# Justin900429/autonomous_driving_with_diffusion_model

Measured on AMD Instinct MI355X. Metric: denoising-steps/sec, higher is better.
Workload: dtype f32

## Files before the change

autonomous_driving_with_diffusion_model_amd/_lib.py:

```python
from __future__ import annotations

import ctypes as C
import os
from typing import Optional, Sequence

import torch

_HERE = os.path.dirname(os.path.abspath(__file__))
LIB_PATH = os.environ.get("ADX_LIB") or os.path.join(_HERE, "libadx.so")

c_f32p = C.POINTER(C.c_float)
i32, i64, f32, vp = C.c_int32, C.c_int64, C.c_float, C.c_void_p


class TConvDesc(C.Structure):
    _fields_ = [("kind", i32), ("taps", i32), ("stride", i32), ("pad", i32), ("c0", i32), ("c1", i32),
                ("cout", i32), ("lin", i32), ("lout", i32), ("groups", i32), ("eps", f32), ("w_layout", i32),
                ("w_flip", i32), ("exact", i32), ("lin_valid", i32), ("lout_valid", i32)]


class TConvIO(C.Structure):
    _fields_ = [("x0", vp), ("x0_sb", i64), ("x0_sc", i64), ("x0_sl", i64),
                ("x1", vp), ("x1_sb", i64), ("x1_sc", i64), ("x1_sl", i64),
                ("packed_w", vp), ("bias", vp), ("gamma", vp), ("beta", vp),
# ... 64 lines not shown
    "adx_resnet_forward": (i32, [vp, vp, vp, vp, i32, i32, i32, vp, vp]),
    "adx_resnet_forward_u8": (i32, [vp, vp, vp, vp, C.POINTER(C.c_float), C.POINTER(C.c_float), i32, i32, i32, vp, vp]),
    "adx_resnet_tape_create": (i32, [C.POINTER(vp)]),
    "adx_resnet_tape_destroy": (None, [vp]),
    "adx_resnet_train_workspace_bytes": (C.c_size_t, [vp, i32, i32, i32]),
    "adx_resnet_forward_train": (i32, [vp, C.POINTER(vp), i32, vp, vp, C.c_size_t, vp, i32, i32, i32, vp, vp, i32, vp]),
    "adx_resnet_backward": (i32, [vp, C.POINTER(vp), C.POINTER(vp), i32, vp, C.c_size_t, vp, vp, vp]),
    "adx_resnet_backward_groups": (i32, [vp]),
    "adx_resnet_tensor_group": (i32, [vp, i32]),
    "adx_resnet_backward_events": (i32, [vp, C.POINTER(vp), C.POINTER(vp), i32, vp, C.c_size_t, vp, vp, C.POINTER(vp), i32, vp]),
    "adx_conv2d_packed_bytes": (C.c_size_t, [C.POINTER(Conv2dDesc)]),
    "adx_conv2d_pack": (i32, [C.POINTER(Conv2dDesc), vp, vp, vp]),
    "adx_conv2d_forward": (i32, [C.POINTER(Conv2dDesc), vp, vp, vp, vp, vp, vp, i32, i32, i32, i32, vp]),
    "adx_conv2d_cells_supported": (i32, [C.POINTER(Conv2dDesc), i32, i32, i32]),
    "adx_conv2d_forward_cells": (i32, [C.POINTER(Conv2dDesc), vp, vp, vp, vp, vp, vp, i32, i32, i32, i32, i32, vp]),
    "adx_conv2d_wgrad_scratch_bytes": (C.c_size_t, []),
    "adx_conv2d_wgrad": (i32, [C.POINTER(Conv2dDesc), vp, vp, vp, i32, i32, i32, vp, vp]),
    "adx_conv2d_wgrad_ex": (i32, [C.POINTER(Conv2dDesc), vp, vp, vp, i32, i32, i32, vp, i32, vp]),
    "adx_conv2d_wgrad_cells": (i32, [C.POINTER(Conv2dDesc), vp, vp, vp, vp, i32, i32, i32, vp, vp]),
    "adx_trajpred_create": (i32, [i32, C.POINTER(vp)]),
    "adx_trajpred_destroy": (None, [vp]),
    "adx_trajpred_num_params": (i32, [vp]),
    "adx_trajpred_packed_bytes": (C.c_size_t, [vp]),
    "adx_trajpred_scratch_bytes": (C.c_size_t, [vp, i32, i32]),
    "adx_trajpred_set_scratch": (i32, [vp, vp, C.c_size_t]),
    "adx_trajpred_pack": (i32, [vp, C.POINTER(vp), i32, vp, vp, vp]),
    "adx_trajpred_forward": (i32, [vp, vp, vp, i64, i64, vp, vp, i32, i32, vp]),
    "adx_trajpred_backward": (i32, [vp, vp, vp, i64, i64, vp, vp, vp, i32, i32, vp]),
    "adx_trajpred_backward_params": (i32, [vp, vp, vp, i64, i64, vp, vp, vp, vp, vp, i32, i32, C.c_float, C.c_uint64, vp]),
    "adx_trajpred_forward_train": (i32, [vp, vp, vp, i64, i64, vp, vp, i32, i32, C.c_float, C.c_uint64, vp]),
# ... 99 lines not shown
```

autonomous_driving_with_diffusion_model_amd/csrc/adx_common.h:

```cpp
#pragma once
#include <atomic>
#include <mutex>
#include <hip/hip_runtime.h>
#include <stdint.h>
#include <stdio.h>
#include <string.h>

#include "../../include/adx.h"

namespace adx {

void set_error(const char* fmt, ...);

#define ADX_CHECK_HIP(expr)                                                              \
  do {                                                                                   \
    hipError_t _e = (expr);                                                              \
    if (_e != hipSuccess) {                                                              \
      adx::set_error("%s failed: %s (%s:%d)", #expr, hipGetErrorString(_e), __FILE__, __LINE__); \
      return ADX_ERR_HIP;                                                                \
    }                                                                                    \
  } while (0)

#define ADX_REQUIRE(cond, ...)                                                           \
  do {                                                                                   \
// ... 14 lines not shown

struct DebugSwitches {
  bool conv_exact = false;
  bool wgrad_exact = false;
  bool tconv_exact = false;
  bool unet_chain = true;
  unsigned chain_mask = ~0u;
  bool unet_pipe = true;
  bool conv_vrow = true;
  bool conv_cells = true;
  int train_cells = 5;
  int hs_mode = -1;
  bool wgrad_deterministic = false;
  bool hs_dma = true;
  bool hs_persist = true;
  int resnet_streams = 2;
  int resnet_split_from = -1;
  bool check_range = false;
};
const DebugSwitches& debug_switches();

struct DeviceOnce {
  std::atomic<uint64_t>& done;
  uint64_t bit = 0;
  bool owner = false;
  static std::mutex& mu() { static std::mutex m; return m; }
  explicit DeviceOnce(std::atomic<uint64_t>& d) : done(d) {
    int dev = 0;
    (void)hipGetDevice(&dev);
    bit = 1ull << (dev & 63);
// ... 38 lines not shown
```

autonomous_driving_with_diffusion_model_amd/csrc/api.cpp:

```cpp
#include <stdarg.h>
#include <stdlib.h>

#include "tconv.h"

namespace adx {

static thread_local char g_err[512] = "";

void set_error(const char* fmt, ...) {
  va_list ap;
  va_start(ap, fmt);
  vsnprintf(g_err, sizeof(g_err), fmt, ap);
  va_end(ap);
}

const DebugSwitches& debug_switches() {
  static const DebugSwitches sw = [] {
    DebugSwitches d;
    auto is = [](const char* name, char v) { const char* e = getenv(name); return e != nullptr && e[0] == v && e[1] == '\0'; };
    d.conv_exact = is("ADX_CONV_EXACT", '1');
    d.wgrad_exact = is("ADX_WGRAD_EXACT", '1');
    d.tconv_exact = is("ADX_TCONV_EXACT", '1');
    d.unet_chain = !is("ADX_UNET_CHAIN", '0');
    d.unet_pipe = !is("ADX_UNET_PIPE", '0');
    d.conv_cells = !is("ADX_CONV_CELLS", '0');
    d.conv_vrow = !is("ADX_CONV_VROW", '0');
    d.train_cells = is("ADX_TRAIN_CELLS", '0') ? 0 : (is("ADX_TRAIN_CELLS", '1') ? 1 : (is("ADX_TRAIN_CELLS", '2') ? 2 : (is("ADX_TRAIN_CELLS", '3') ? 3 : (is("ADX_TRAIN_CELLS", '4') ? 4 : 5))));
    d.check_range = is("ADX_CHECK_RANGE", '1');
    d.hs_dma = !is("ADX_HS_DMA", '0');
    d.hs_persist = !is("ADX_HS_PERSIST", '0');
    d.wgrad_deterministic = is("ADX_WGRAD_DETERMINISTIC", '1');
    if (const char* e = getenv("ADX_CHAIN_MASK")) d.chain_mask = (unsigned)strtoul(e, nullptr, 0);
    if (const char* e = getenv("ADX_HS_MODE")) d.hs_mode = atoi(e);
    if (const char* e = getenv("ADX_RESNET_SPLIT_FROM")) d.resnet_split_from = atoi(e) < 0 ? -1 : atoi(e);
    if (const char* e = getenv("ADX_RESNET_STREAMS")) d.resnet_streams = atoi(e) < 1 ? 1 : (atoi(e) > 4 ? 4 : atoi(e));
    return d;
  }();
  return sw;
}

int embed_forward(const adx_embed_weights* w, int dim, const int64_t* t, int t_rows, const float* cond,
                  const float* feat, int feat_rows, int rows, float* time_embed, float* mish_cond, hipStream_t s);
int ddim_step(const adx_step_coef* c, const float* mo, const float* x, const float* z, const float* tgt,
              const float* mask, float* prev, float* x0, int b, int h, int d, hipStream_t s);
int ddpm_step(const adx_step_coef* c, const float* mo, const float* x, const float* z, const float* tgt,
// ... 58 lines not shown
```

autonomous_driving_with_diffusion_model_amd/csrc/conv2d.hip:

```cpp
#include <stdlib.h>

#include <vector>

#include "adx_common.h"
#include "conv2d_internal.h"

namespace adx {

constexpr int kCoutT = 64;
constexpr size_t kMaxLds = 96 * 1024;
constexpr int g_conv_cc = 16;
constexpr int g_conv_rows = 2;

template <int STRIDE, int K, int ROWS, int CCH = 16>
__global__ void __launch_bounds__(256) conv2d_kernel(const Conv2dArgs a) {
  constexpr int TH = 4 * ROWS;
  constexpr int CC = (K == 7) ? 4 : CCH;
  constexpr int PH = (TH - 1) * STRIDE + K;
  constexpr int PW = (kTileW - 1) * STRIDE + K;
  constexpr int PLANE = PH * PW;
  constexpr int NP = CC * PLANE;
  constexpr int PITEMS = (NP + 255) / 256;
  constexpr int NTAPS = K * K;
  constexpr int NW4 = NTAPS * CC * (kCoutT / 4);
// ... 465 lines not shown
}

int adx_conv2d_forward_cells(const adx_conv2d_desc* d, const void* x, const float* packed_w, const float* scale,
                             const float* shift, const void* res, void* y, int32_t n, int32_t h, int32_t w, int32_t relu,
                             int32_t fmt, adx_stream stream) {
  ConvSpec L;
  int rc = spec_from_desc(d, &L);
  if (rc != ADX_OK) return rc;
  ADX_REQUIRE(x && packed_w && y, "adx_conv2d_forward_cells: null tensor");
  ADX_REQUIRE((scale == nullptr) == (shift == nullptr), "adx_conv2d_forward_cells: scale and shift go together");
  ADX_REQUIRE(fmt >= 0 && fmt <= 7 && (fmt & kFmtYCells), "adx_conv2d_forward_cells: fmt %d (the output is a cell tensor)", fmt);
  ADX_REQUIRE(conv2d_hs3x3_plain(L, n, h, w), "adx_conv2d_forward_cells: not a plain launch of the pipelined 3x3 kernel "
              "(adx_conv2d_cells_supported)");
  return conv2d_launch_raw(L, (const float*)x, packed_w, scale, shift, (const float*)res, (float*)y, n, h, w, relu,
                           (hipStream_t)stream, nullptr, 0, nullptr, 0, nullptr, fmt);
}

int adx_resnet_create(int32_t out_dim, adx_resnet** out) {
  ADX_REQUIRE(out != nullptr && out_dim >= 1 && out_dim <= 4096, "adx_resnet_create: bad argument");
  adx_resnet* r = new adx_resnet();
  r->out_dim = out_dim;
  int t = 0;
  size_t off = 0;
  auto add = [&](int cin, int cout, int k, int stride, int pad) {
    ConvSpec L{};
    L.cin = cin; L.cout = cout; L.k = k; L.stride = stride; L.pad = pad;
    L.t_w = t++; L.t_g = t++; L.t_b = t++; L.t_m = t++; L.t_v = t++;
    L.cc = cin >= 16 ? 16 : 4;
    L.cin_pad = round_up(cin, L.cc);
    L.fuse_with = -1;
// ... 314 lines not shown
```

autonomous_driving_with_diffusion_model_amd/csrc/conv2d_hs.hip:

```cpp
#include <type_traits>
#include <stdlib.h>

#include "adx_common.h"
#include "conv2d_internal.h"
#include "conv2d_hs_common.h"

namespace adx {

template <bool AFFINE = true>
__device__ __forceinline__ void cells_store32(float (&v)[16], const float* sc, const float* sh, int cl0, const float (*res8)[8],
                                              bool relu, __amdgpu_buffer_rsrc_t yrsrc, uint32_t vcell, uint32_t so, uint32_t cplane) {
#pragma unroll
  for (int i = 0; i < 2; ++i)
#pragma unroll
    for (int j = 0; j < 4; ++j) {
      const auto sw = __builtin_amdgcn_permlane32_swap(f2u(v[8 * i + j]), f2u(v[8 * i + 4 + j]), false, false);
      v[8 * i + j] = u2f(sw[0]);
      v[8 * i + 4 + j] = u2f(sw[1]);
    }
#pragma unroll
  for (int i = 0; i < 2; ++i) {
    float o[8];
#pragma unroll
    for (int j = 0; j < 8; ++j) {
// ... 1319 lines not shown
  if (frames_u8 != nullptr) {
    ADX_REQUIRE(mean && stdv, "conv2d_hs_stem_pool: uint8 frames need mean / std");
    a.x_u8 = frames_u8;
    for (int c = 0; c < 3; ++c) { a.u8_mean[c] = mean[c]; a.u8_std[c] = stdv[c]; }
  }
  a.N = N; a.Cin = 3; a.H = H; a.W = W; a.Cout = 64;
  a.OH = conv_out_dim(H, 7, 2, 3); a.OW = conv_out_dim(W, 7, 2, 3);
  a.KH = 7; a.KW = 7; a.stride = 2; a.pad = 3; a.relu = 1;
  a.cin_pad = L.cin_pad; a.cc = L.cc;
  a.y_cells = y_cells;
  return frames_u8 != nullptr ? hs_stem_launch<true, true>(a, s) : hs_stem_launch<true>(a, s);
}

int conv2d_hs_launch_block_s2(const ConvSpec& c1, const ConvSpec& ds, const float* x, const float* w1, const float* scale1,
                              const float* shift1, float* y1, const float* wd, const float* scaled, const float* shiftd,
                              float* yd, int N, int H, int W, hipStream_t s, int x_cells, int y_cells, int relu) {
  ADX_REQUIRE(x && w1 && y1 && wd && yd && (scale1 != nullptr) == (shift1 != nullptr) && (scaled != nullptr) == (shiftd != nullptr),
              "conv2d_hs block launch: null pointer");
  Conv2dArgs a{};
  a.x = x; a.w = w1; a.scale = scale1; a.shift = shift1; a.res = nullptr; a.y = y1; a.x_amax = nullptr; a.x_amax_n = 0;
  a.w_ds = wd; a.scale_ds = scaled; a.shift_ds = shiftd; a.y_ds = yd;
  a.N = N; a.Cin = c1.cin; a.H = H; a.W = W; a.Cout = c1.cout;
  a.OH = conv_out_dim(H, 3, 2, 1); a.OW = conv_out_dim(W, 3, 2, 1);
  a.KH = 3; a.KW = 3; a.stride = 2; a.pad = 1; a.relu = relu;
  a.cin_pad = c1.cin_pad; a.cc = c1.cc;
  a.x_cells = x_cells;
  a.y_cells = y_cells;
  (void)ds;
  return conv2d_hs_launch(c1, a, s);
}

__global__ void __launch_bounds__(256) conv2d_split_reduce_kernel(const float* __restrict__ part, size_t part_stride, int nparts,
                                                                  const float* __restrict__ scale, const float* __restrict__ shift,
                                                                  const float* __restrict__ res, float* __restrict__ y,
                                                                  int cout, int plane4, size_t total4, int relu) {
  const size_t i = (size_t)blockIdx.x * 256 + threadIdx.x;
  if (i >= total4) return;
  const int c = (int)((i / plane4) % cout);
  f32x4 v = reinterpret_cast<const f32x4*>(part)[i];
  for (int p0 = 1; p0 < nparts; p0 += 8) {
    f32x4 t[8];
#pragma unroll
    for (int j = 0; j < 8; ++j) t[j] = reinterpret_cast<const f32x4*>(part + (size_t)(p0 + j < nparts ? p0 + j : 0) * part_stride)[i];
// ... 258 lines not shown
  ConvSpec g{};
  g.cin = cout; g.cin_pad = cout; g.cout = 4 * cin; g.k = 2; g.stride = 1; g.pad = 0; g.cc = kHsCC;
  int rc = conv2d_hs_pack(g, wbuild, wimg, 0, s);
  if (rc != ADX_OK) return rc;
  Conv2dArgs a{};
  a.x = dy; a.w = wimg; a.res = accumulate ? dx : nullptr; a.y = dx; a.x_amax = dy_amax; a.x_amax_n = dy_amax_n;
  a.N = N; a.Cin = cout; a.H = conv_out_dim(H, 3, 2, 1); a.W = conv_out_dim(W, 3, 2, 1); a.Cout = 4 * cin;
  a.OH = a.H; a.OW = a.W;
  a.KH = 2; a.KW = 2; a.stride = 1; a.pad = 0; a.relu = 0;
  a.cin_pad = cout; a.cc = kHsCC;
  a.d2s_cin = cin; a.d2s_h = H; a.d2s_w = W;
  ADX_REQUIRE((size_t)cin * H * W * sizeof(float) < 0x7FFFFFFFu, "conv2d_hs_dgrad_s2: one image of dx exceeds the 32-bit byte offsets");
  return hs_launch_t<1, 2, 2, 2, false>(a, s);
}

int conv2d_hs_launch(const ConvSpec& L, Conv2dArgs a, hipStream_t s) {
  ADX_REQUIRE((size_t)L.cin * a.H * a.W * sizeof(float) < 0xC0000000u, "conv2d_hs: one image of the input exceeds the 32-bit byte offsets");
  const bool ds = a.w_ds != nullptr;
  if (hs_is_stem(L) && !ds) {
    ADX_REQUIRE(a.x_amax == nullptr && a.res == nullptr, "conv2d_hs stem: no residual / dynamic range");
    return hs_stem_launch<false>(a, s);
  }
  if (L.k == 3 && L.stride == 1 && !ds) {
    const int mode = hs3x3_mode(L, a);
    if (mode >= 0) return mode == 1 ? hs3x3_launch<1>(a, s) : (mode == 2 ? hs3x3_launch<2>(a, s) : hs3x3_launch<0>(a, s));
    ADX_REQUIRE(a.stats_part == nullptr, "conv2d_hs: statistics requested from a launch the pipelined kernel does not serve");
    return hs_launch_t<1, 3, 2, 2, false>(a, s);
  }
  if (L.k == 3 && L.stride == 2 && L.pad == 1) {
    if (a.x_cells || a.y_cells) {
      ADX_REQUIRE(ds && a.x_amax == nullptr && a.res == nullptr && a.d2s_cin == 0,
                  "conv2d_hs: cell-layout operands of the stride-2 conv need the fused downsample launch (no residual, no dynamic range)");
      if (a.x_cells && a.y_cells) return hs_launch_t<2, 3, 1, 1, true, true, true>(a, s);
      return a.x_cells ? hs_launch_t<2, 3, 1, 1, true, true, false>(a, s) : hs_launch_t<2, 3, 1, 1, true, false, true>(a, s);
    }
    return ds ? hs_launch_t<2, 3, 1, 1, true>(a, s) : hs_launch_t<2, 3, 1, 1, false>(a, s);
  }
  set_error("conv2d_hs: no kernel for k=%d stride=%d pad=%d%s", L.k, L.stride, L.pad, ds ? " with a fused downsample" : "");
  return ADX_ERR_INVALID;
}

}

#ifdef ADX_HS_TRACE
extern "C" int adx_hs_trace_read(unsigned long long* host, int nwords) {
  return (int)hipMemcpyFromSymbol(host, HIP_SYMBOL(adx::g_hs_trace), (size_t)nwords * 8);
}
#endif
// ... 1 lines not shown
```

autonomous_driving_with_diffusion_model_amd/csrc/conv2d_hs16.hip:

```cpp
#include "adx_common.h"
#include "conv2d_internal.h"
#include "conv2d_hs_common.h"

namespace adx {

namespace {

constexpr int kQNT = 512;
constexpr int kQTH = 8;
constexpr int kQPW = 34;
constexpr int kQPlane = (kQTH + 2) * kQPW;
constexpr int kQPlaneP = 344;
constexpr int kQPairs = 4 * kQPlane;
constexpr int kQPit = (kQPairs + kQNT - 1) / kQNT;
constexpr int kQWst = 1024;
constexpr size_t kQLds = (size_t)2 * 8 * kQPlaneP * 16 + (size_t)2 * kQWst * 16 + 256 * sizeof(float) + 2 * 16 + 512 * sizeof(float);
constexpr int kQPlaneD = 352;
constexpr int kQPairsD = 4 * kQPlaneD;
constexpr size_t kQLdsD = (size_t)2 * 8 * kQPlaneD * 16 + (size_t)2 * kQWst * 16 + 256 * sizeof(float) + 2 * 16 + 512 * sizeof(float) +
                          (size_t)kQPit * kQNT * sizeof(uint32_t);
typedef __attribute__((address_space(3))) void lds_void;

__device__ __forceinline__ f32x4 mfma16(f16x8 a, f16x8 b, f32x4 c) { return __builtin_amdgcn_mfma_f32_16x16x32_f16(a, b, c, 0, 0, 0); }

__device__ __forceinline__ void half4(uint32_t h0, uint32_t h1, uint32_t l0, uint32_t l1, float* out) {
  const float inv = 1.f / kLoScale;
  asm("v_fma_mix_f32 %0, %1, %2, %3 op_sel:[0,0,0] op_sel_hi:[1,0,1]" : "=v"(out[0]) : "v"(l0), "s"(inv), "v"(h0));
  asm("v_fma_mix_f32 %0, %1, %2, %3 op_sel:[1,0,1] op_sel_hi:[1,0,1]" : "=v"(out[1]) : "v"(l0), "s"(inv), "v"(h0));
  asm("v_fma_mix_f32 %0, %1, %2, %3 op_sel:[0,0,0] op_sel_hi:[1,0,1]" : "=v"(out[2]) : "v"(l1), "s"(inv), "v"(h1));
  asm("v_fma_mix_f32 %0, %1, %2, %3 op_sel:[1,0,1] op_sel_hi:[1,0,1]" : "=v"(out[3]) : "v"(l1), "s"(inv), "v"(h1));
}

}

template <bool DMA, int TRAIN = 0>
__global__ void __launch_bounds__(kQNT, 2) conv2d_hs3x3q_kernel(const Conv2dArgs a) {
// ... 479 lines not shown
    ADX_CHECK_HIP(hipFuncSetAttribute(reinterpret_cast<const void*>(&conv2d_hs3x3q_kernel<true, 2>), hipFuncAttributeMaxDynamicSharedMemorySize, (int)kQLdsD));
    once.commit();
  }
  a.vw = a.N > 1 ? a.OW + 1 : a.OW;
  a.inv_vw = 1.f / (float)a.vw;
  ADX_REQUIRE((long)a.N * a.vw < (1L << 21), "conv2d_hs: batch x width exceeds the virtual-row arithmetic");
  a.tiles_x = ceil_div(a.N * a.vw - (a.N > 1 ? 1 : 0), 32);
  a.tiles_y = ceil_div(a.OH, kQTH);
  a.cout_tiles = a.Cout / 128;
  const size_t tiles = (size_t)a.cout_tiles * a.tiles_x * a.tiles_y;
  ADX_REQUIRE(tiles < (1u << 31), "conv2d_hs: grid too large");
  a.ntiles = (int)tiles;
  const int nsp = a.tiles_x * a.tiles_y;
  int slots = ceil_div(nsp, 8);
  if (debug_switches().hs_dma && debug_switches().hs_persist) {
    static std::atomic<int> n_cu{0};
    int cus = n_cu.load(std::memory_order_relaxed);
    if (cus == 0) {
      int dev = 0;
      hipDeviceProp_t prop;
      ADX_CHECK_HIP(hipGetDevice(&dev));
      ADX_CHECK_HIP(hipGetDeviceProperties(&prop, dev));
      cus = prop.multiProcessorCount > 8 ? prop.multiProcessorCount : 8;
      n_cu.store(cus, std::memory_order_relaxed);
    }
    slots = std::min(slots, std::max(1, cus / (8 * a.cout_tiles)));
  }
  a.q_slots = slots;
  const size_t grid = (size_t)8 * a.cout_tiles * slots;
  ADX_REQUIRE((size_t)a.N * a.Cout * a.OH * a.OW * sizeof(float) < 0xC0000000u && (size_t)a.N * a.Cin * a.H * a.W * sizeof(float) < 0xC0000000u,
              "conv2d_hs: a cell-layout tensor exceeds the 32-bit byte offsets");
  if (train) {
    ADX_REQUIRE(a.stats_p == a.tiles_y * a.tiles_x, "conv2d_hs3x3q: statistics buffer laid out for %d tiles, launch has %d", a.stats_p,
                a.tiles_y * a.tiles_x);
    if (dgrad) {
      if (debug_switches().hs_dma) conv2d_hs3x3q_kernel<true, 2><<<dim3((unsigned)grid), dim3(kQNT), kQLdsD, s>>>(a);
      else conv2d_hs3x3q_kernel<false, 2><<<dim3((unsigned)grid), dim3(kQNT), kQLds, s>>>(a);
    } else if (debug_switches().hs_dma) conv2d_hs3x3q_kernel<true, 1><<<dim3((unsigned)grid), dim3(kQNT), kQLdsD, s>>>(a);
    else conv2d_hs3x3q_kernel<false, 1><<<dim3((unsigned)grid), dim3(kQNT), kQLds, s>>>(a);
  } else if (debug_switches().hs_dma) conv2d_hs3x3q_kernel<true><<<dim3((unsigned)grid), dim3(kQNT), kQLdsD, s>>>(a);
  else conv2d_hs3x3q_kernel<false><<<dim3((unsigned)grid), dim3(kQNT), kQLds, s>>>(a);
  ADX_LAUNCH_CHECK();
  return ADX_OK;
}

}
```

autonomous_driving_with_diffusion_model_amd/csrc/conv2d_internal.h:

```cpp
#pragma once
#include <vector>

#include "adx_common.h"

namespace adx {

constexpr int kTileH = 4;
constexpr int kTileW = 32;

struct ConvSpec {
  int cin, cout, k, stride, pad;
  int t_w, t_g, t_b, t_m, t_v;
  size_t o_w, o_scale, o_shift;
  int cin_pad, cc;
  int fuse_with;
  int dgrad;
};

struct Conv2dArgs {
  const float* x;
  const float* w;
  const float* scale;
  const float* shift;
  const float* res;
// ... 60 lines not shown
bool conv2d_hs3x3_dgrad_stats(const ConvSpec& L, int N, int H, int W, bool x_cells, size_t stats_floats);
bool conv2d_hs3x3q_train_eligible(const Conv2dArgs& a);
bool conv2d_hs3x3q_dgrad_eligible(const Conv2dArgs& a);
int conv2d_hs3x3q_train_tiles(const Conv2dArgs& a);
int conv2d_pack_raw(const float* w, float* packed, int cout, int cin, int k, int cin_pad, int dgrad, hipStream_t s);
int conv2d_pack_spec(const ConvSpec& consumer, const float* w, float* packed, int dgrad, hipStream_t s);
bool conv2d_hs_eligible(const ConvSpec& L);
size_t conv2d_packed_floats(const ConvSpec& L);
int conv2d_hs_pack(const ConvSpec& consumer, const float* w, void* packed, int dgrad, hipStream_t s);
struct HsPackJob { const float* w; void* packed; int cout, cin_pad, cin, taps, dgrad; };
bool conv2d_hs_pack_batchable(const ConvSpec& consumer, int dgrad);
int conv2d_hs_pack_many(const HsPackJob* jobs, int n, hipStream_t s);
int conv2d_hs_launch(const ConvSpec& L, Conv2dArgs a, hipStream_t s);
bool conv2d_hs3x3q_eligible(const Conv2dArgs& a);
int conv2d_hs3x3q_launch(Conv2dArgs a, hipStream_t s);
int conv2d_hs_stats_tiles(const ConvSpec& L, const Conv2dArgs& a);
bool conv2d_hs_dgrad_s2_eligible(int cin, int cout);
int conv2d_hs_dgrad_s2(const float* w, const float* dy, float* dx, int accumulate, int N, int cin, int cout, int H, int W,
                       float* wbuild, float* wimg, const uint32_t* dy_amax, int dy_amax_n, hipStream_t s);
void conv2d_set_split_scratch(float* p, size_t floats);
int conv2d_hs_stem_pool(const ConvSpec& L, const float* x, const float* w, const float* scale, const float* shift,
                        float* pooled, int N, int H, int W, hipStream_t s, const uint8_t* frames_u8 = nullptr,
                        const float* mean = nullptr, const float* stdv = nullptr, int y_cells = 0);
int conv2d_hs_launch_block_s2(const ConvSpec& c1, const ConvSpec& ds, const float* x, const float* w1, const float* scale1,
                              const float* shift1, float* y1, const float* wd, const float* scaled, const float* shiftd,
                              float* yd, int N, int H, int W, hipStream_t s, int x_cells = 0, int y_cells = 0, int relu = 1);
inline bool resnet_fuses_ds(const ConvSpec& c1, const ConvSpec& ds) {
  return conv2d_hs_eligible(c1) && c1.k == 3 && c1.stride == 2 && c1.pad == 1 && ds.k == 1 && ds.stride == 2 && ds.pad == 0 &&
         ds.cin == c1.cin && ds.cout == c1.cout;
}
bool conv2d_wgrad_hs_eligible(int Cin, int Cout, int k, int stride, int pad);
int conv2d_wgrad_hs(const float* x, const float* dy, float* dw, int N, int Cin, int H, int W, int Cout, int stride,
                    const uint32_t* dy_amax, int dy_amax_n, hipStream_t s, bool x_cells = false, bool dy_cells = false);
void conv2d_wgrad_set_partials(float* p, size_t floats);
size_t conv2d_wgrad_partials_floats();
bool conv2d_wgrad_stem_hs_eligible(int Cin, int Cout, int k, int stride, int pad);
int conv2d_wgrad_stem_hs(const float* x, const float* dy, float* dw, int N, int H, int W, const uint32_t* dy_amax, int dy_amax_n,
                         hipStream_t s);
inline int conv_out_dim(int h, int k, int s, int p) { return (h + 2 * p - k) / s + 1; }
int conv2d_range_check(const char* what, int index, const float* t, size_t floats, bool cells, hipStream_t s);
int maxpool_launch(const float* x, float* y, int planes, int H, int W, int OH, int OW, hipStream_t s);
// ... 5 lines not shown
```

autonomous_driving_with_diffusion_model_amd/ops.py:

```python
from __future__ import annotations

import ctypes as C
import math
import os
from typing import Optional

import torch

from . import _lib as L


def _strides3(t: torch.Tensor):
    return t.stride(0), t.stride(1), t.stride(2)


def tconv(x0: torch.Tensor, weight: torch.Tensor, bias: Optional[torch.Tensor] = None, *, x1: Optional[torch.Tensor] = None,
          kind: int = 0, stride: int = 1, pad: int = 0, gn_weight: Optional[torch.Tensor] = None,
          gn_bias: Optional[torch.Tensor] = None, groups: int = 0, eps: float = 1e-5,
          tbias: Optional[torch.Tensor] = None, res: Optional[torch.Tensor] = None,
          out: Optional[torch.Tensor] = None, scratch: Optional[torch.Tensor] = None,
          tickets: Optional[torch.Tensor] = None) -> torch.Tensor:
    assert x0.is_cuda and x0.dtype == torch.float32 and x0.dim() == 3
    B, c0, lin = x0.shape
    c1 = 0 if x1 is None else x1.shape[1]
# ... 103 lines not shown

def conv2d_cells(x: torch.Tensor, packed: torch.Tensor, cin: int, cout: int, n: int, h: int, w: int, *, x_cells: bool,
                 scale=None, shift=None, res=None, res_cells: bool = False, relu: bool = False,
                 out: Optional[torch.Tensor] = None) -> torch.Tensor:
    d = L.Conv2dDesc(cin, cout, 3, 1, 1)
    if not L.lib().adx_conv2d_cells_supported(C.byref(d), n, h, w):
        raise ValueError(f"conv2d_cells: {cin}->{cout} at {n}x{h}x{w} is not a plain launch of the pipelined 3x3 kernel")
    y = out if out is not None else torch.empty(n * cout * h * w * 4, dtype=torch.uint8, device=x.device)
    fmt = (1 if x_cells else 0) | 2 | (4 if (res is not None and res_cells) else 0)
    L.check(L.lib().adx_conv2d_forward_cells(C.byref(d), x.data_ptr(), packed.data_ptr(), L.ptr(scale), L.ptr(shift), L.ptr(res),
                                             y.data_ptr(), n, h, w, int(relu), fmt, L.stream_ptr(x.device)),
            "adx_conv2d_forward_cells")
    return y


def conv2d_weight_grad(x: torch.Tensor, dy: torch.Tensor, k: int, *, stride: int = 1, pad: int = 0,
                       estimate_range: bool = True) -> torch.Tensor:
    assert x.is_cuda and dy.is_cuda and x.dtype == dy.dtype == torch.float32 and x.is_contiguous() and dy.is_contiguous()
    n, cin, h, w = x.shape
    cout = dy.shape[1]
    d = L.Conv2dDesc(cin, cout, k, stride, pad)
    dw = torch.empty((cout, cin, k, k), dtype=torch.float32, device=x.device)
    scratch = torch.empty(L.lib().adx_conv2d_wgrad_scratch_bytes(), dtype=torch.uint8, device=x.device)
    L.check(L.lib().adx_conv2d_wgrad_ex(C.byref(d), x.data_ptr(), dy.data_ptr(), dw.data_ptr(), n, h, w, scratch.data_ptr(),
                                        int(bool(estimate_range)), L.stream_ptr(x.device)), "adx_conv2d_wgrad_ex")
    return dw


def conv2d_weight_grad_cells(x: torch.Tensor, dy: torch.Tensor) -> torch.Tensor:
    assert x.is_cuda and dy.is_cuda and x.dtype == dy.dtype == torch.float32
# ... 30 lines not shown
```

include/adx.h:

```cpp
#ifndef ADX_H
#define ADX_H

#include <stddef.h>
#include <stdint.h>

#ifdef __cplusplus
extern "C" {
#endif

#define ADX_OK 0
#define ADX_ERR_INVALID (-1)
#define ADX_ERR_HIP (-2)
#define ADX_ERR_STATE (-3)
#define ADX_ERR_RANGE (-4)

typedef void* adx_stream;

int adx_version(void);
const char* adx_source_hash(void);
const char* adx_last_error(void);


typedef struct adx_tconv_desc {
  int32_t kind, taps, stride, pad;
// ... 100 lines not shown
                       int32_t batch, int32_t h, int32_t w, float* feature , adx_stream s);
int adx_resnet_forward_u8(adx_resnet* r, const void* packed, void* workspace, const uint8_t* frames_hwc,
                          const float* mean , const float* stdv , int32_t batch, int32_t h, int32_t w,
                          float* feature , adx_stream s);

typedef struct adx_conv2d_desc { int32_t cin, cout, k, stride, pad; } adx_conv2d_desc;
size_t adx_conv2d_packed_bytes(const adx_conv2d_desc* d);
int adx_conv2d_pack(const adx_conv2d_desc* d, const float* w , float* packed, adx_stream s);
int adx_conv2d_forward(const adx_conv2d_desc* d, const float* x, const float* packed_w, const float* scale,
                       const float* shift, const float* res, float* y, int32_t n, int32_t h, int32_t w,
                       int32_t relu, adx_stream s);
int adx_conv2d_cells_supported(const adx_conv2d_desc* d, int32_t n, int32_t h, int32_t w);
int adx_conv2d_forward_cells(const adx_conv2d_desc* d, const void* x, const float* packed_w, const float* scale,
                             const float* shift, const void* res, void* y, int32_t n, int32_t h, int32_t w, int32_t relu,
                             int32_t fmt, adx_stream s);
size_t adx_conv2d_wgrad_scratch_bytes(void);
int adx_conv2d_wgrad(const adx_conv2d_desc* d, const float* x, const float* dy, float* dw, int32_t n, int32_t h,
                     int32_t w, void* scratch, adx_stream s);
int adx_conv2d_wgrad_ex(const adx_conv2d_desc* d, const float* x, const float* dy, float* dw, int32_t n, int32_t h,
                        int32_t w, void* scratch, int32_t estimate_range, adx_stream s);
int adx_conv2d_wgrad_cells(const adx_conv2d_desc* d, const void* x_cells, const void* dy_cells, const float* dy_scale, float* dw,
                           int32_t n, int32_t h, int32_t w, void* scratch, adx_stream s);

typedef struct adx_resnet_tape adx_resnet_tape;
int adx_resnet_tape_create(adx_resnet_tape** out);
void adx_resnet_tape_destroy(adx_resnet_tape* t);
size_t adx_resnet_train_workspace_bytes(const adx_resnet* r, int32_t batch, int32_t h, int32_t w);
int adx_resnet_forward_train(adx_resnet* r, const float* const* tensors, int32_t n_tensors, void* packed,
                             void* workspace, size_t workspace_bytes, const float* img, int32_t batch, int32_t h,
                             int32_t w, float* feature, adx_resnet_tape* tape, int32_t update_running, adx_stream s);
// ... 91 lines not shown
```

Measured before the change: 167.4.

## Add persistent pipelined stride-2 3x3 conv kernel with fused downsample

```diff
diff --git a/autonomous_driving_with_diffusion_model_amd/_lib.py b/autonomous_driving_with_diffusion_model_amd/_lib.py
--- a/autonomous_driving_with_diffusion_model_amd/_lib.py
+++ b/autonomous_driving_with_diffusion_model_amd/_lib.py
@@ -102,6 +102,8 @@
     "adx_conv2d_forward": (i32, [C.POINTER(Conv2dDesc), vp, vp, vp, vp, vp, vp, i32, i32, i32, i32, vp]),
     "adx_conv2d_cells_supported": (i32, [C.POINTER(Conv2dDesc), i32, i32, i32]),
     "adx_conv2d_forward_cells": (i32, [C.POINTER(Conv2dDesc), vp, vp, vp, vp, vp, vp, i32, i32, i32, i32, i32, vp]),
+    "adx_conv2d_block_s2_pack": (i32, [i32, i32, vp, vp, vp, vp, vp]),
+    "adx_conv2d_block_s2_cells": (i32, [i32, i32, vp, vp, vp, vp, vp, vp, vp, vp, vp, i32, i32, i32, i32, vp]),
     "adx_conv2d_wgrad_scratch_bytes": (C.c_size_t, []),
     "adx_conv2d_wgrad": (i32, [C.POINTER(Conv2dDesc), vp, vp, vp, i32, i32, i32, vp, vp]),
     "adx_conv2d_wgrad_ex": (i32, [C.POINTER(Conv2dDesc), vp, vp, vp, i32, i32, i32, vp, i32, vp]),
diff --git a/autonomous_driving_with_diffusion_model_amd/csrc/adx_common.h b/autonomous_driving_with_diffusion_model_amd/csrc/adx_common.h
--- a/autonomous_driving_with_diffusion_model_amd/csrc/adx_common.h
+++ b/autonomous_driving_with_diffusion_model_amd/csrc/adx_common.h
@@ -52,6 +52,7 @@
   bool wgrad_deterministic = false;
   bool hs_dma = true;
   bool hs_persist = true;
+  bool hs_s2 = true;
   int resnet_streams = 2;
   int resnet_split_from = -1;
   bool check_range = false;
diff --git a/autonomous_driving_with_diffusion_model_amd/csrc/api.cpp b/autonomous_driving_with_diffusion_model_amd/csrc/api.cpp
--- a/autonomous_driving_with_diffusion_model_amd/csrc/api.cpp
+++ b/autonomous_driving_with_diffusion_model_amd/csrc/api.cpp
@@ -29,6 +29,7 @@
     d.check_range = is("ADX_CHECK_RANGE", '1');
     d.hs_dma = !is("ADX_HS_DMA", '0');
     d.hs_persist = !is("ADX_HS_PERSIST", '0');
+    d.hs_s2 = !is("ADX_HS_S2", '0');
     d.wgrad_deterministic = is("ADX_WGRAD_DETERMINISTIC", '1');
     if (const char* e = getenv("ADX_CHAIN_MASK")) d.chain_mask = (unsigned)strtoul(e, nullptr, 0);
     if (const char* e = getenv("ADX_HS_MODE")) d.hs_mode = atoi(e);
diff --git a/autonomous_driving_with_diffusion_model_amd/csrc/conv2d.hip b/autonomous_driving_with_diffusion_model_amd/csrc/conv2d.hip
--- a/autonomous_driving_with_diffusion_model_amd/csrc/conv2d.hip
+++ b/autonomous_driving_with_diffusion_model_amd/csrc/conv2d.hip
@@ -503,6 +503,37 @@
               "(adx_conv2d_cells_supported)");
   return conv2d_launch_raw(L, (const float*)x, packed_w, scale, shift, (const float*)res, (float*)y, n, h, w, relu,
                            (hipStream_t)stream, nullptr, 0, nullptr, 0, nullptr, fmt);
+}
+
+static int block_s2_specs(int32_t cin, int32_t cout, ConvSpec* c1, ConvSpec* ds) {
+  adx_conv2d_desc d1{cin, cout, 3, 2, 1}, dd{cin, cout, 1, 2, 0};
+  int rc = spec_from_desc(&d1, c1);
+  if (rc == ADX_OK) rc = spec_from_desc(&dd, ds);
+  if (rc != ADX_OK) return rc;
+  ADX_REQUIRE(resnet_fuses_ds(*c1, *ds), "adx_conv2d_block_s2: %d -> %d is not a fused split-fp16 block entry", cin, cout);
+  return ADX_OK;
+}
+
+int adx_conv2d_block_s2_pack(int32_t cin, int32_t cout, const float* w1, const float* wd, float* packed1, float* packed_ds,
+                             adx_stream stream) {
+  ConvSpec c1, ds;
+  int rc = block_s2_specs(cin, cout, &c1, &ds);
+  if (rc != ADX_OK) return rc;
+  ADX_REQUIRE(w1 && wd && packed1 && packed_ds, "adx_conv2d_block_s2_pack: null pointer");
+  rc = conv2d_hs_pack(c1, w1, packed1, 0, (hipStream_t)stream);
+  return rc != ADX_OK ? rc : conv2d_hs_pack(ds, wd, packed_ds, 0, (hipStream_t)stream);
+}
+
+int adx_conv2d_block_s2_cells(int32_t cin, int32_t cout, const void* x, const float* packed1, const float* scale1, const float* shift1,
+                              void* y1, const float* packed_ds, const float* scaled, const float* shiftd, void* yd, int32_t n, int32_t h,
+                              int32_t w, int32_t kernel, adx_stream stream) {
+  ConvSpec c1, ds;
+  int rc = block_s2_specs(cin, cout, &c1, &ds);
+  if (rc != ADX_OK) return rc;
+  ADX_REQUIRE(x && packed1 && y1 && packed_ds && yd, "adx_conv2d_block_s2_cells: null tensor");
+  ADX_REQUIRE(n >= 1 && h >= 2 && w >= 2 && cin % 8 == 0 && kernel >= 0 && kernel <= 3, "adx_conv2d_block_s2_cells: bad argument");
+  return conv2d_hs_launch_block_s2(c1, ds, (const float*)x, packed1, scale1, shift1, (float*)y1, packed_ds, scaled, shiftd, (float*)yd,
+                                   n, h, w, (hipStream_t)stream, 1, 1, 1, kernel);
 }
 
 int adx_resnet_create(int32_t out_dim, adx_resnet** out) {
diff --git a/autonomous_driving_with_diffusion_model_amd/csrc/conv2d_hs.hip b/autonomous_driving_with_diffusion_model_amd/csrc/conv2d_hs.hip
--- a/autonomous_driving_with_diffusion_model_amd/csrc/conv2d_hs.hip
+++ b/autonomous_driving_with_diffusion_model_amd/csrc/conv2d_hs.hip
@@ -1357,7 +1357,7 @@
 
 int conv2d_hs_launch_block_s2(const ConvSpec& c1, const ConvSpec& ds, const float* x, const float* w1, const float* scale1,
                               const float* shift1, float* y1, const float* wd, const float* scaled, const float* shiftd,
-                              float* yd, int N, int H, int W, hipStream_t s, int x_cells, int y_cells, int relu) {
+                              float* yd, int N, int H, int W, hipStream_t s, int x_cells, int y_cells, int relu, int kernel) {
   ADX_REQUIRE(x && w1 && y1 && wd && yd && (scale1 != nullptr) == (shift1 != nullptr) && (scaled != nullptr) == (shiftd != nullptr),
               "conv2d_hs block launch: null pointer");
   Conv2dArgs a{};
@@ -1370,6 +1370,12 @@
   a.x_cells = x_cells;
   a.y_cells = y_cells;
   (void)ds;
+  if (kernel != 0) {
+    ADX_REQUIRE(x_cells && y_cells && kernel >= 1 && kernel <= 3 && conv2d_hs_eligible(c1) && a.cin_pad % kHsCC == 0,
+                "conv2d_hs block launch: kernel %d needs cell tensors in and out", kernel);
+    if (kernel == 1) return hs_launch_t<2, 3, 1, 1, true, true, true>(a, s);
+    return conv2d_hs3x3s2q_launch(a, s, kernel == 2 ? 1 : 0);
+  }
   return conv2d_hs_launch(c1, a, s);
 }
 
@@ -1658,6 +1664,8 @@
   return hs_launch_t<1, 2, 2, 2, false>(a, s);
 }
 
+constexpr int kS2qMinTiles = 128;
+
 int conv2d_hs_launch(const ConvSpec& L, Conv2dArgs a, hipStream_t s) {
   ADX_REQUIRE((size_t)L.cin * a.H * a.W * sizeof(float) < 0xC0000000u, "conv2d_hs: one image of the input exceeds the 32-bit byte offsets");
   const bool ds = a.w_ds != nullptr;
@@ -1675,7 +1683,11 @@
     if (a.x_cells || a.y_cells) {
       ADX_REQUIRE(ds && a.x_amax == nullptr && a.res == nullptr && a.d2s_cin == 0,
                   "conv2d_hs: cell-layout operands of the stride-2 conv need the fused downsample launch (no residual, no dynamic range)");
-      if (a.x_cells && a.y_cells) return hs_launch_t<2, 3, 1, 1, true, true, true>(a, s);
+      if (a.x_cells && a.y_cells) {
+        if (debug_switches().hs_s2 && a.Cin >= 128 && conv2d_hs3x3s2q_eligible(a) && conv2d_hs3x3s2q_tiles(a) >= kS2qMinTiles)
+          return conv2d_hs3x3s2q_launch(a, s, debug_switches().hs_persist ? 1 : 0);
+        return hs_launch_t<2, 3, 1, 1, true, true, true>(a, s);
+      }
       return a.x_cells ? hs_launch_t<2, 3, 1, 1, true, true, false>(a, s) : hs_launch_t<2, 3, 1, 1, true, false, true>(a, s);
     }
     return ds ? hs_launch_t<2, 3, 1, 1, true>(a, s) : hs_launch_t<2, 3, 1, 1, false>(a, s);
diff --git a/autonomous_driving_with_diffusion_model_amd/csrc/conv2d_hs16.hip b/autonomous_driving_with_diffusion_model_amd/csrc/conv2d_hs16.hip
--- a/autonomous_driving_with_diffusion_model_amd/csrc/conv2d_hs16.hip
+++ b/autonomous_driving_with_diffusion_model_amd/csrc/conv2d_hs16.hip
@@ -20,6 +20,25 @@
 constexpr size_t kQLdsD = (size_t)2 * 8 * kQPlaneD * 16 + (size_t)2 * kQWst * 16 + 256 * sizeof(float) + 2 * 16 + 512 * sizeof(float) +
                           (size_t)kQPit * kQNT * sizeof(uint32_t);
 typedef __attribute__((address_space(3))) void lds_void;
+
+static_assert(kQLds <= 160 * 1024 && kQLdsD <= 160 * 1024, "one workgroup per CU: LDS holds 160 KiB");
+
+hipError_t device_cus(int* out) {
+  static std::atomic<int> n_cu[64] = {};
+  int dev = 0;
+  hipError_t e = hipGetDevice(&dev);
+  if (e != hipSuccess) return e;
+  int cus = n_cu[dev & 63].load(std::memory_order_relaxed);
+  if (cus == 0) {
+    hipDeviceProp_t prop;
+    e = hipGetDeviceProperties(&prop, dev);
+    if (e != hipSuccess) return e;
+    cus = prop.multiProcessorCount > 8 ? prop.multiProcessorCount : 8;
+    n_cu[dev & 63].store(cus, std::memory_order_relaxed);
+  }
+  *out = cus;
+  return hipSuccess;
+}
 
 __device__ __forceinline__ f32x4 mfma16(f16x8 a, f16x8 b, f32x4 c) { return __builtin_amdgcn_mfma_f32_16x16x32_f16(a, b, c, 0, 0, 0); }
 
@@ -529,16 +548,8 @@
   const int nsp = a.tiles_x * a.tiles_y;
   int slots = ceil_div(nsp, 8);
   if (debug_switches().hs_dma && debug_switches().hs_persist) {
-    static std::atomic<int> n_cu{0};
-    int cus = n_cu.load(std::memory_order_relaxed);
-    if (cus == 0) {
-      int dev = 0;
-      hipDeviceProp_t prop;
-      ADX_CHECK_HIP(hipGetDevice(&dev));
-      ADX_CHECK_HIP(hipGetDeviceProperties(&prop, dev));
-      cus = prop.multiProcessorCount > 8 ? prop.multiProcessorCount : 8;
-      n_cu.store(cus, std::memory_order_relaxed);
-    }
+    int cus = 0;
+    ADX_CHECK_HIP(device_cus(&cus));
     slots = std::min(slots, std::max(1, cus / (8 * a.cout_tiles)));
   }
   a.q_slots = slots;
@@ -559,4 +570,286 @@
   return ADX_OK;
 }
 
-}
+namespace {
+constexpr int kSNT = 512;
+constexpr int kSTH = 4;
+constexpr int kSPW = 65;
+constexpr int kSEvn = 33;
+constexpr int kSPE = 336;
+constexpr int kSPO = 272;
+constexpr int kSPiecesE = kSPE * 4 / 64;
+constexpr int kSPiecesO = kSPO * 4 / 64;
+constexpr int kSRounds = 3;
+constexpr int kSWst = 1024;
+constexpr size_t kSLds = (size_t)2 * 4 * (kSPE + kSPO) * 16 + (size_t)4 * kSWst * 16 + 4 * 128 * sizeof(float);
+static_assert(kSLds <= 160 * 1024, "one workgroup per CU: LDS holds 160 KiB");
+static_assert(kSPiecesE <= 8 * kSRounds && kSPiecesO <= 8 * kSRounds, "three rounds of 8 waves stage a region");
+}
+
+__global__ void __launch_bounds__(kSNT, 2) conv2d_hs3x3s2q_kernel(const Conv2dArgs a) {
+  constexpr int NT = kSNT, PW = kSPW, WST = kSWst;
+  extern __shared__ __attribute__((aligned(16))) unsigned char smem_raw[];
+  u32x4* pe = reinterpret_cast<u32x4*>(smem_raw);
+  u32x4* po = pe + 2 * 4 * kSPE;
+  u32x4* wl = po + 2 * 4 * kSPO;
+  u32x4* wds = wl + 3 * WST;
+  float* ss = reinterpret_cast<float*>(wds + WST);
+  const int tid = threadIdx.x, lane = tid & 63;
+  const int wave = __builtin_amdgcn_readfirstlane(tid >> 6);
+  const int row = wave & 3, slab = wave >> 2;
+  const int j = lane & 15, kq = lane >> 4;
+  const int Qs = a.q_slots;
+  const int xcd = blockIdx.x & 7, rr_ = blockIdx.x >> 3;
+  const int ct = rr_ % a.cout_tiles, slot = rr_ / a.cout_tiles;
+  const int nsp = a.tiles_x * a.tiles_y;
+  const int sp_end = (int)(((long)(xcd + 1) * nsp) >> 3);
+  int sp = (int)(((long)xcd * nsp) >> 3) + slot;
+  if (sp >= sp_end) return;
+  int ty = sp / a.tiles_x, tx = sp - ty * a.tiles_x;
+  auto vdiv = [&](int v) { return (int)(((float)v + 0.5f) * a.inv_vw); };
+  const size_t hw = (size_t)a.H * a.W;
+  const int nch16 = a.cin_pad / 16, nch32 = a.cin_pad / 32, nstages = nch32 * 9;
+  constexpr uint32_t kOutside = 0xC0000000u;
+  const __amdgpu_buffer_rsrc_t xrsrc = __builtin_amdgcn_make_buffer_rsrc(
+      const_cast<float*>(a.x), 0, (int)(uint32_t)((size_t)a.N * a.Cin * hw * sizeof(float)), 0x00020000);
+  const uint32_t plane_bytes = (uint32_t)(hw * sizeof(float));
+  auto goff_of = [&](int k, bool odd, int ty_, int tx_) -> uint32_t {
+    const int P = odd ? kSPO : kSPE, nrows = odd ? 4 : 5;
+    const int e = tid + NT * k;
+    const int g = e / P, p = e - g * P;
+    const int prow = p / PW, pc = p - prow * PW;
+    const int py = 2 * prow + (odd ? 1 : 0);
+    const int px = pc < kSEvn ? 2 * pc : 2 * (pc - kSEvn) + 1;
+    const int iy = 2 * ty_ * kSTH - 1 + py;
+    const int q = tx_ * 32 + (px >> 1);
+    const int ni = vdiv(q);
+    const int ix = 2 * (q - ni * a.vw) + (px & 1) - 1;
+    const bool ok = p < nrows * PW && iy >= 0 && iy < a.H && ix >= 0 && ix < a.W && ni < a.N;
+    return !ok ? kOutside : (uint32_t)((size_t)ni * a.Cin * hw * sizeof(float) + (size_t)g * 8 * hw * sizeof(float) + ((size_t)iy * a.W + ix) * 16);
+  };
+  const u32x4* wsrc = reinterpret_cast<const u32x4*>(a.w);
+  const u32x4* dsrc = reinterpret_cast<const u32x4*>(a.w_ds);
+  int wsrc_off[2], dsrc_off[2];
+#pragma unroll
+  for (int k = 0; k < 2; ++k) {
+    const int e = tid + NT * k;
+    const int sl = e >> 9, half16 = (e >> 8) & 1, within = e & 255;
+    wsrc_off[k] = (((ct * 2 + sl) * nch16 + half16) * 9) * 256 + within;
+    dsrc_off[k] = ((ct * 2 + sl) * nch16 + half16) * 256 + within;
+  }
+  const int wcell = __builtin_amdgcn_readfirstlane(tid & ~63);
+  auto load_w = [&](int stage, int buf) {
+    const int chunk = stage / 9, i = stage - chunk * 9;
+    const int kh = i < 3 ? 1 : (i < 6 ? 0 : 2), tap = kh * 3 + i % 3;
+    const u32x4* ws = wsrc + (size_t)(chunk * 18 + tap) * 256;
+#pragma unroll
+    for (int k = 0; k < 2; ++k) __builtin_amdgcn_global_load_lds(ws + wsrc_off[k], (lds_void*)(wl + buf * WST + wcell + NT * k), 16, 0, 0);
+  };
+  auto load_ds = [&](int chunk) {
+    const u32x4* ws = dsrc + (size_t)chunk * 512;
+#pragma unroll
+    for (int k = 0; k < 2; ++k) __builtin_amdgcn_global_load_lds(ws + dsrc_off[k], (lds_void*)(wds + wcell + NT * k), 16, 0, 0);
+  };
+  auto load_p = [&](bool odd, int chunk, int k, uint32_t go) {
+    const int P = odd ? kSPO : kSPE;
+    if (wave + 8 * k < (odd ? kSPiecesO : kSPiecesE)) {
+      const uint32_t cbase = (uint32_t)chunk * 32u * plane_bytes;
+      u32x4* d = (odd ? po : pe) + wcell + NT * k;
+      __builtin_amdgcn_raw_ptr_buffer_load_lds(xrsrc, (lds_void*)d, 16, go, cbase, 0, 0);
+      __builtin_amdgcn_raw_ptr_buffer_load_lds(xrsrc, (lds_void*)(d + 4 * P), 16, go, cbase + 4 * plane_bytes, 0, 0);
+    }
+  };
+
+  uint32_t goe[kSRounds], goc[kSRounds], goo[kSRounds];
+#pragma unroll
+  for (int k = 0; k < kSRounds; ++k) goo[k] = goff_of(k, true, ty, tx);
+  load_w(0, 0);
+  load_w(1, 1);
+  load_ds(0);
+#pragma unroll
+  for (int k = 0; k < kSRounds; ++k) load_p(true, 0, k, goo[k]);
+  {
+    const int which = tid >> 7, c = ct * 128 + (tid & 127);
+    const float* src = which == 0 ? a.scale : (which == 1 ? a.shift : (which == 2 ? a.scale_ds : a.shift_ds));
+    ss[tid] = src == nullptr ? ((which & 1) == 0 ? 1.f : 0.f) : src[c];
+  }
+  asm volatile("s_waitcnt vmcnt(0)" ::: "memory");
+  __syncthreads();
+
+  f32x4 accm[4][2], accl[4][2], dsm[4][2], dsl[4][2];
+  for (;;) {
+    const int oy0 = ty * kSTH, vx0 = tx * 32;
+    const int sp_next = sp + Qs;
+    const bool has_next = sp_next < sp_end;
+    const int nty = sp_next / a.tiles_x, ntx = sp_next - nty * a.tiles_x;
+#pragma unroll
+    for (int k = 0; k < kSRounds; ++k) {
+      goe[k] = goff_of(k, false, ty, tx);
+      goc[k] = goff_of(k, true, ty, tx);
+      goo[k] = has_next ? goff_of(k, true, nty, ntx) : kOutside;
+    }
+#pragma unroll
+    for (int cb = 0; cb < 4; ++cb)
+#pragma unroll
+      for (int pb = 0; pb < 2; ++pb)
+#pragma unroll
+        for (int i = 0; i < 4; ++i) { accm[cb][pb][i] = 0.f; accl[cb][pb][i] = 0.f; dsm[cb][pb][i] = 0.f; dsl[cb][pb][i] = 0.f; }
+    const int wa_lane = slab * 512 + (kq >> 1) * 256 + (kq & 1) * 64 + j;
+
+    for (int c = 0; c < nch32; ++c) {
+      const bool last = c + 1 == nch32;
+#pragma unroll 1
+      for (int i = 0; i < 9; ++i) {
+        const int s = 9 * c + i;
+        const int kh = i < 3 ? 1 : (i < 6 ? 0 : 2), kw = i % 3;
+        if (i < 3) load_p(false, c, i, i == 0 ? goe[0] : (i == 1 ? goe[1] : goe[2]));
+        else if (i < 6) {
+          if (!last) load_p(true, c + 1, i - 3, i == 3 ? goc[0] : (i == 4 ? goc[1] : goc[2]));
+          else if (has_next) load_p(true, 0, i - 3, i == 3 ? goo[0] : (i == 4 ? goo[1] : goo[2]));
+        }
+        if (i == 2) {
+          if (!last) load_ds(c + 1);
+          else if (has_next) load_ds(0);
+        }
+        load_w(s + 2 < nstages ? s + 2 : s + 2 - nstages, (i + 2) % 3);
+        __builtin_amdgcn_sched_barrier(0);
+        const u32x4* wa0 = wl + (i % 3) * WST + wa_lane;
+        const int P = kh == 1 ? kSPO : kSPE;
+        const u32x4* pb0 = (kh == 1 ? po + row * PW : pe + (row + (kh >> 1)) * PW) + kq * P + j + (kw & 1) * kSEvn + (kw >> 1);
+        f16x8 A[2][4], B[2][2];
+#pragma unroll
+        for (int pl = 0; pl < 2; ++pl) {
+#pragma unroll
+          for (int cb = 0; cb < 4; ++cb) A[pl][cb] = __builtin_bit_cast(f16x8, wa0[pl * 128 + cb * 16]);
+#pragma unroll
+          for (int pb = 0; pb < 2; ++pb) B[pl][pb] = __builtin_bit_cast(f16x8, pb0[pl * 4 * P + pb * 16]);
+        }
+#pragma unroll
+        for (int pb = 0; pb < 2; ++pb) {
+#pragma unroll
+          for (int cb = 0; cb < 4; ++cb) {
+            accm[cb][pb] = mfma16(A[0][cb], B[0][pb], accm[cb][pb]);
+            accl[cb][pb] = mfma16(A[0][cb], B[1][pb], accl[cb][pb]);
+          }
+#pragma unroll
+          for (int cb = 0; cb < 4; ++cb) accl[cb][pb] = mfma16(A[1][cb], B[0][pb], accl[cb][pb]);
+        }
+        if (i == 1) {
+          f16x8 D[2][4];
+#pragma unroll
+          for (int pl = 0; pl < 2; ++pl)
+#pragma unroll
+            for (int cb = 0; cb < 4; ++cb) D[pl][cb] = __builtin_bit_cast(f16x8, wds[wa_lane + pl * 128 + cb * 16]);
+#pragma unroll
+          for (int pb = 0; pb < 2; ++pb) {
+#pragma unroll
+            for (int cb = 0; cb < 4; ++cb) {
+              dsm[cb][pb] = mfma16(D[0][cb], B[0][pb], dsm[cb][pb]);
+              dsl[cb][pb] = mfma16(D[0][cb], B[1][pb], dsl[cb][pb]);
+            }
+#pragma unroll
+            for (int cb = 0; cb < 4; ++cb) dsl[cb][pb] = mfma16(D[1][cb], B[0][pb], dsl[cb][pb]);
+          }
+        }
+        asm volatile("s_waitcnt vmcnt(2)" ::: "memory");
+        __syncthreads();
+      }
+    }
+
+    {
+      const int vcol = vx0 + 16 * (kq & 1) + j;
+      const int nl = vdiv(vcol), xl = vcol - nl * a.vw;
+      const int oy = oy0 + row;
+      const uint32_t plane_ob = (uint32_t)(a.OH * a.OW) * (uint32_t)sizeof(float);
+      const uint32_t cplane = (uint32_t)(a.OH * a.OW) * 16u;
+      const uint32_t img_bytes = (uint32_t)a.N * (uint32_t)a.Cout * plane_ob;
+      const int cout0 = ct * 128 + slab * 64;
+      const uint32_t cell0 = (uint32_t)(cout0 >> 3) * 2u * cplane;
+      const uint32_t vcell = (nl < a.N && xl < a.OW && oy < a.OH)
+                                 ? (uint32_t)nl * (uint32_t)a.Cout * plane_ob + (uint32_t)(oy * a.OW + xl) * 16u + (uint32_t)(kq >> 1) * 2u * cplane
+                                 : kOutside;
+#pragma unroll
+      for (int br = 0; br < 2; ++br) {
+        const float* sc = ss + 256 * br + slab * 64;
+        const float* sh = sc + 128;
+        const __amdgpu_buffer_rsrc_t orsrc = __builtin_amdgcn_make_buffer_rsrc(br == 0 ? a.y : a.y_ds, 0, (int)img_bytes, 0x00020000);
+        const bool relu = br == 0 && a.relu != 0;
+#pragma unroll
+        for (int cb = 0; cb < 4; ++cb) {
+          float x[4], y[4];
+#pragma unroll
+          for (int i = 0; i < 4; ++i) {
+            const int cl = cb * 16 + 4 * kq + i;
+            const f32x4 m0 = br == 0 ? accm[cb][0] : dsm[cb][0], l0 = br == 0 ? accl[cb][0] : dsl[cb][0];
+            const f32x4 m1 = br == 0 ? accm[cb][1] : dsm[cb][1], l1 = br == 0 ? accl[cb][1] : dsl[cb][1];
+            x[i] = (m0[i] + l0[i] * (1.f / kLoScale)) * sc[cl] + sh[cl];
+            y[i] = (m1[i] + l1[i] * (1.f / kLoScale)) * sc[cl] + sh[cl];
+          }
+          float o[8];
+#pragma unroll
+          for (int i = 0; i < 4; ++i) {
+            const auto sw = __builtin_amdgcn_permlane16_swap(f2u(x[i]), f2u(y[i]), false, false);
+            o[i] = u2f(sw[0]);
+            o[4 + i] = u2f(sw[1]);
+          }
+#pragma unroll
+          for (int i = 0; i < 8; ++i) o[i] = relu ? __builtin_fmaxf(o[i], 0.f) : o[i];
+          u32x4 hi, lo;
+          split8(o, 1.f, hi, lo);
+          const uint32_t so = cell0 + (uint32_t)(2 * cb) * 2u * cplane;
+          __builtin_amdgcn_raw_buffer_store_b128(hi, orsrc, vcell, so, 0);
+          __builtin_amdgcn_raw_buffer_store_b128(lo, orsrc, vcell, so + cplane, 0);
+          asm volatile("s_nop 0" ::"v"(hi), "v"(lo));
+        }
+      }
+    }
+    if (!has_next) {
+      asm volatile("s_waitcnt vmcnt(0)" ::: "memory");
+      break;
+    }
+    sp = sp_next; tx = ntx; ty = nty;
+  }
+}
+
+bool conv2d_hs3x3s2q_eligible(const Conv2dArgs& a) {
+  if (!(a.x_cells && a.y_cells && a.w_ds != nullptr && a.y_ds != nullptr && a.res == nullptr && a.x_amax == nullptr &&
+        a.stats_part == nullptr && a.d2s_cin == 0 && a.Cout % 128 == 0 && a.cin_pad % 64 == 0 && a.cin_pad == a.Cin && a.pad == 1 &&
+        a.stride == 2 && a.KH == 3 && a.KW == 3 && a.OH == (a.H - 1) / 2 + 1 && a.OW == (a.W - 1) / 2 + 1 && a.N >= 1))
+    return false;
+  const long vw = a.OW + 1;
+  return a.N * vw + 64 < (1L << 21) && (size_t)a.N * a.Cout * a.OH * a.OW * sizeof(float) < 0xC0000000u &&
+         (size_t)a.N * a.Cin * a.H * a.W * sizeof(float) < 0xC0000000u;
+}
+
+int conv2d_hs3x3s2q_tiles(const Conv2dArgs& a) {
+  return (a.Cout / 128) * ceil_div(a.OH, kSTH) * ceil_div(a.N * (a.OW + 1) - 1, 32);
+}
+
+int conv2d_hs3x3s2q_launch(Conv2dArgs a, hipStream_t s, int persist) {
+  ADX_REQUIRE(conv2d_hs3x3s2q_eligible(a), "conv2d_hs3x3s2q: launch outside the kernel's rules");
+  static std::atomic<uint64_t> attr{0};
+  if (DeviceOnce once{attr}; once) {
+    ADX_CHECK_HIP(hipFuncSetAttribute(reinterpret_cast<const void*>(&conv2d_hs3x3s2q_kernel), hipFuncAttributeMaxDynamicSharedMemorySize, (int)kSLds));
+    once.commit();
+  }
+  a.vw = a.OW + 1;
+  a.inv_vw = 1.f / (float)a.vw;
+  a.tiles_x = ceil_div(a.N * a.vw - 1, 32);
+  a.tiles_y = ceil_div(a.OH, kSTH);
+  a.cout_tiles = a.Cout / 128;
+  a.ntiles = a.cout_tiles * a.tiles_x * a.tiles_y;
+  const int nsp = a.tiles_x * a.tiles_y;
+  int slots = ceil_div(nsp, 8);
+  if (persist) {
+    int cus = 0;
+    ADX_CHECK_HIP(device_cus(&cus));
+    slots = std::min(slots, std::max(1, cus / (8 * a.cout_tiles)));
+  }
+  a.q_slots = slots;
+  const size_t grid = (size_t)8 * a.cout_tiles * slots;
+  conv2d_hs3x3s2q_kernel<<<dim3((unsigned)grid), dim3(kSNT), kSLds, s>>>(a);
+  ADX_LAUNCH_CHECK();
+  return ADX_OK;
+}
+
+}
diff --git a/autonomous_driving_with_diffusion_model_amd/csrc/conv2d_internal.h b/autonomous_driving_with_diffusion_model_amd/csrc/conv2d_internal.h
--- a/autonomous_driving_with_diffusion_model_amd/csrc/conv2d_internal.h
+++ b/autonomous_driving_with_diffusion_model_amd/csrc/conv2d_internal.h
@@ -98,6 +98,9 @@
 int conv2d_hs_launch(const ConvSpec& L, Conv2dArgs a, hipStream_t s);
 bool conv2d_hs3x3q_eligible(const Conv2dArgs& a);
 int conv2d_hs3x3q_launch(Conv2dArgs a, hipStream_t s);
+bool conv2d_hs3x3s2q_eligible(const Conv2dArgs& a);
+int conv2d_hs3x3s2q_tiles(const Conv2dArgs& a);
+int conv2d_hs3x3s2q_launch(Conv2dArgs a, hipStream_t s, int persist);
 int conv2d_hs_stats_tiles(const ConvSpec& L, const Conv2dArgs& a);
 bool conv2d_hs_dgrad_s2_eligible(int cin, int cout);
 int conv2d_hs_dgrad_s2(const float* w, const float* dy, float* dx, int accumulate, int N, int cin, int cout, int H, int W,
@@ -108,7 +111,8 @@
                         const float* mean = nullptr, const float* stdv = nullptr, int y_cells = 0);
 int conv2d_hs_launch_block_s2(const ConvSpec& c1, const ConvSpec& ds, const float* x, const float* w1, const float* scale1,
                               const float* shift1, float* y1, const float* wd, const float* scaled, const float* shiftd,
-                              float* yd, int N, int H, int W, hipStream_t s, int x_cells = 0, int y_cells = 0, int relu = 1);
+                              float* yd, int N, int H, int W, hipStream_t s, int x_cells = 0, int y_cells = 0, int relu = 1,
+                              int kernel = 0);
 inline bool resnet_fuses_ds(const ConvSpec& c1, const ConvSpec& ds) {
   return conv2d_hs_eligible(c1) && c1.k == 3 && c1.stride == 2 && c1.pad == 1 && ds.k == 1 && ds.stride == 2 && ds.pad == 0 &&
          ds.cin == c1.cin && ds.cout == c1.cout;
diff --git a/autonomous_driving_with_diffusion_model_amd/ops.py b/autonomous_driving_with_diffusion_model_amd/ops.py
--- a/autonomous_driving_with_diffusion_model_amd/ops.py
+++ b/autonomous_driving_with_diffusion_model_amd/ops.py
@@ -141,6 +141,29 @@
     return y
 
 
+def block_s2_pack(w1: torch.Tensor, wd: torch.Tensor):
+    cout, cin = w1.shape[:2]
+    w1 = w1.detach().contiguous()
+    wd = wd.detach().reshape(cout, cin).contiguous()
+    p1 = torch.empty(9 * cin * cout, dtype=torch.float32, device=w1.device)
+    pd = torch.empty(cin * cout, dtype=torch.float32, device=w1.device)
+    L.check(L.lib().adx_conv2d_block_s2_pack(cin, cout, w1.data_ptr(), wd.data_ptr(), p1.data_ptr(), pd.data_ptr(),
+                                             L.stream_ptr(w1.device)), "adx_conv2d_block_s2_pack")
+    return p1, pd
+
+
+def block_s2_cells(x: torch.Tensor, p1: torch.Tensor, pd: torch.Tensor, cin: int, cout: int, n: int, h: int, w: int, *,
+                   scale1=None, shift1=None, scaled=None, shiftd=None, kernel: int = 0, out=None):
+    oh, ow = (h - 1) // 2 + 1, (w - 1) // 2 + 1
+    nbytes = n * cout * oh * ow * 4
+    y1, yd = out if out is not None else (torch.empty(nbytes, dtype=torch.uint8, device=x.device),
+                                          torch.empty(nbytes, dtype=torch.uint8, device=x.device))
+    L.check(L.lib().adx_conv2d_block_s2_cells(cin, cout, x.data_ptr(), p1.data_ptr(), L.ptr(scale1), L.ptr(shift1), y1.data_ptr(),
+                                              pd.data_ptr(), L.ptr(scaled), L.ptr(shiftd), yd.data_ptr(), n, h, w, int(kernel),
+                                              L.stream_ptr(x.device)), "adx_conv2d_block_s2_cells")
+    return y1, yd
+
+
 def conv2d_weight_grad(x: torch.Tensor, dy: torch.Tensor, k: int, *, stride: int = 1, pad: int = 0,
                        estimate_range: bool = True) -> torch.Tensor:
     assert x.is_cuda and dy.is_cuda and x.dtype == dy.dtype == torch.float32 and x.is_contiguous() and dy.is_contiguous()
diff --git a/include/adx.h b/include/adx.h
--- a/include/adx.h
+++ b/include/adx.h
@@ -138,6 +138,11 @@
 int adx_conv2d_forward_cells(const adx_conv2d_desc* d, const void* x, const float* packed_w, const float* scale,
                              const float* shift, const void* res, void* y, int32_t n, int32_t h, int32_t w, int32_t relu,
                              int32_t fmt, adx_stream s);
+int adx_conv2d_block_s2_pack(int32_t cin, int32_t cout, const float* w1, const float* wd, float* packed1, float* packed_ds,
+                             adx_stream s);
+int adx_conv2d_block_s2_cells(int32_t cin, int32_t cout, const void* x, const float* packed1, const float* scale1, const float* shift1,
+                              void* y1, const float* packed_ds, const float* scaled, const float* shiftd, void* yd, int32_t n, int32_t h,
+                              int32_t w, int32_t kernel, adx_stream s);
 size_t adx_conv2d_wgrad_scratch_bytes(void);
 int adx_conv2d_wgrad(const adx_conv2d_desc* d, const float* x, const float* dy, float* dw, int32_t n, int32_t h,
                      int32_t w, void* scratch, adx_stream s);
```

New measurement: 166.6, median of 6. No clear change (-0.5%).
